# acados/acados

Measured on NVIDIA H100. Metric: OCP-QP solves/sec (fp64, batch) chain-mass N=40, higher is better.
Workload: dtype f64

## Files before the change

### acados_b200/csrc/cuipm_fast_core.h

```cpp
#ifndef CUIPM_FAST_CORE_H_
#define CUIPM_FAST_CORE_H_

#include "cuipm_device.h"

#ifndef FK_PROF_T0
#define FK_PROF_T0() do {} while (0)
#define FK_PROF_ADD(slot) do {} while (0)
#define FK_PROF_T2() do {} while (0)
#define FK_PROF_ADD2(slot) do {} while (0)
#endif

#define FK_FOR_SLACK(i, jj) \
    _Pragma("unroll 1") for (int i_ = inv[jj], i = i_ >= 0 ? i_ : 0, e_ = i_ >= 0 ? i_ + 1 : (i_ == -2 ? nb : 0); i < e_; i++) \
        if (i_ >= 0 || rev[i] == (jj))

#define FK_PRAGMA_(x) _Pragma(#x)
#define FK_PRAGMA(x) FK_PRAGMA_(x)
#ifndef FK_VLOOP_N
#define FK_VLOOP_N 1
#endif
#define FK_VLOOP FK_PRAGMA(unroll FK_VLOOP_N)
#ifndef FK_TILE_N
#define FK_TILE_LOOP _Pragma("unroll")
#else
// ... 10 lines not shown
#ifndef FK_U_TRMM
#define FK_U_TRMM 4
#endif
#ifndef FK_U_SYRK
#define FK_U_SYRK 3
#endif
#ifndef FK_U_UPD
#define FK_U_UPD 2
#endif

namespace cuipm {
namespace fastk {

FK_DEV int evn(int n) { return (n + 1) & ~1; }

struct QpState
{
    double mu, obj, gap, alpha, res_m_tau;
    double res_max[4];
};

template <int NX, int NU, int G>
struct Ker
{
    static constexpr int NM = NX + NU;
    static constexpr int QPW = 32 / G;
    static constexpr int LDK = NM | 1;
    static constexpr int LDW = ((NM + 1) / 4) * 4 + 2;
    static constexpr int RPM = (NM + G - 1) / G;
    static constexpr int NXe = (NX + 1) & ~1, NMe = (NM + 2) & ~1;
    static constexpr int SZA = (LDK * NX + 1) & ~1;
    static constexpr int SZL = LDW * NM;
    static constexpr int SZU = (NM * NU + 1) & ~1;
    static constexpr int SZD = 0;
// ... 131 lines not shown
    }
    FK_DEV void st(double *p, double v) const { if (act) *p = v; }
    template <bool ALIGNED>
    FK_DEV fk_double2 ld_pair(const double *p) const
    {
        if (ALIGNED) return fk_ld2(p);
        fk_double2 r;
        r.x = p[0]; r.y = p[1];
        return r;
    }

    template <int REC, int BAR>
    FK_DEV void bulk(int soff, size_t off, int nd, int pf = 0)
    {
        if (li == 0)
            fk_bulk(smem0 + (size_t) gq * A.gstride + soff, (REC == 0 ? qk : (REC == 1 ? sol : (REC == 2 ? wk : qp))) + off, (unsigned) nd * 8u, bars + BAR);
        (void) pf;
        if (BAR == 0) tx0 += (unsigned) (QPW * nd) * 8u;
        else tx1 += (unsigned) (QPW * nd) * 8u;
    }
    template <int REC>
    FK_DEV void vcopy(double *dst, size_t off, int nd)
    {
        const double *src = (REC == 0 ? qk : (REC == 1 ? sol : (REC == 2 ? wk : qp))) + off;
FK_VLOOP
        for (int e = 2 * li; e < nd; e += 2 * G) fk_cp16(dst + e, src + e);
    }
    FK_DEV void stage_begin() { fk_fence_async(); fk_sync(); }
    FK_DEV void stage_arm()
    {
        if (fk_lane() == 0) fk_mbar_arrive_tx(bars + 1, tx1);
        tx1 = 0;
    }
    FK_DEV void stage_arm_vec() {}
    FK_DEV void stage_arm_mat()
    {
        if (fk_lane() == 0) fk_mbar_arrive_tx(bars + 1, tx1);
        tx1 = 0;
    }
    FK_DEV void wait_vec() { FK_PROF_T0(); fk_cp_wait(); fk_sync(); FK_PROF_ADD(5); }
    FK_DEV void wait_mat() { FK_PROF_T0(); fk_mbar_wait(bars + 1, ph1); ph1 ^= 1u; FK_PROF_ADD(6); }
// ... 91 lines not shown

    FK_DEV void res_issue_mat(int k)
    {
        const StageDesc &s = sdr(k);
        const unsigned kk = (k >= 1 && k < A.N) ? (unsigned) (k - 1) : 0u;
        const int kind = k == 0 ? 0 : (k == A.N ? 2 : 1);
        if (s.nx1 > 0) bulk<0, 1>(voff(MA), (size_t) A.kq[kind] + (size_t) kk * A.kqs, evn(LDK * s.nx1));
        bulk<0, 1>(voff(ML), (size_t) A.kq[kind] + (size_t) kk * A.kqs + A.kH[kind], evn(LDK * s.n));
        stage_arm_mat();
    }

    struct ResAcc
    {
        double a_mu, a_obj, a_gap, m0, m1, m2, m3, m4;
        int f0, f1, f2, f3, f4;
    };

    template <int KIND>
    FK_DEV void res_stage(int k, int update, double alpha_u, ResAcc &R)
    {
        constexpr int nx = KD<KIND>::nx, nu = KD<KIND>::nu, n = nx + nu, nx1 = KD<KIND>::nx1;
        constexpr int RP = (n + G - 1) / G, CP = (nx1 + G - 1) / G;
        const StageDesc &sd = sdk<KIND>();
        const View v = view<KIND>(k);
        const int nb = sd.nb, ns = sd.ns, nc = sd.nc;
        const int *idxb = IDX + 4 * (A.nmaps == 3 ? KIND : k) * A.nbe, *rev = idxb + nb, *inv = rev + nb;
        const int nu1 = (nx1 > 0 && k + 1 < A.N) ? NU : 0, n1e = (nx1 + nu1 + 1) & ~1;
        const int solN = (int) (sd.sol.t - sd.sol.ux) + evn(nc), stpN = (int) (sd.step.t - sd.step.ux) + evn(nc);
        const int qvN = (int) ((sd.q_stage + sd.q_stage_bytes / 8u) - sd.q_b);
        double *SOL = V, *STP = SOL + (A.nve + NXe + 2 * A.nce), *SOLN = STP + (A.nve + NXe + 2 * A.nce), *STPN = SOLN + NMe;
        double *QV = STPN + NMe, *tmp0 = QV + (NXe + NMe + 2 * A.nce + 2 * A.ns2e), *tmp1 = tmp0 + A.nbe, *g_ = tmp1 + A.nbe, *pim = g_ + A.nve;
        double *x1 = pim + NXe;
        const int pf = (KIND == 1 && k + 1 < A.N) ? 1 : 0;
        stage_begin();
        vcopy<1>(SOL, (size_t) v.kk * A.ss + sd.sol.ux, solN);
        if (update) vcopy<2>(STP, (size_t) v.kk * A.ws + sd.step.ux, stpN);
        vcopy<0>(QV, (size_t) A.kq[KIND] + (size_t) v.kk * A.kqs + A.kV[KIND], evn(qvN));
        if (nx1 > 0)
        {
            const StageDesc &s1 = sdr(k + 1);
            const View v1 = viewr(k + 1);
            vcopy<1>(SOLN, (size_t) v1.kk * A.ss + s1.sol.ux, n1e);
            if (update) vcopy<2>(STPN, (size_t) v1.kk * A.ws + s1.step.ux, n1e);
        }
        stage_arm_vec();
        if (KIND == 0) res_issue_mat(k);
        wait_vec();
        double *ux = SOL, *pi = SOL + (sd.sol.pi - sd.sol.ux), *lam = SOL + (sd.sol.lam - sd.sol.ux), *t = SOL + (sd.sol.t - sd.sol.ux);
        const double *du = STP, *dp = STP + (sd.step.pi - sd.step.ux), *dl = STP + (sd.step.lam - sd.step.ux), *dtt = STP + (sd.step.t - sd.step.ux);
        const double *qb = QV, *qrq = QV + (sd.q_rq - sd.q_b), *qd = QV + (sd.q_d - sd.q_b), *msk = QV + (sd.q_dmask - sd.q_b);
        const double *qZ = QV + (sd.q_Z - sd.q_b), *qz = QV + (sd.q_z - sd.q_b);
        if (update)
// ... 36 lines not shown
                        tt = tt <= A.o.t_min ? A.o.t_min : tt;
                    }
                    l *= mk;
                    st(gl + i, l);
                    st(gt + i, tt);
                }
                lam[i] = l * mk;
                t[i] = tt;
            }
        }
        fk_sync();
FK_VLOOP
        for (int i = li; i < nb; i += G) tmp0[i] = lam[nb + i] - lam[i];
        wait_mat();
        fk_sync();
        {
            double hx[RPM > 0 ? RPM : 1], ap[RPM > 0 ? RPM : 1];
            rows_dot<n, n>(ML, LDK, ux, hx);
            if (nx1 > 0) rows_dot<n, nx1>(MA, LDK, pi, ap);
#pragma unroll
            for (int m = 0; m < RP; m++)
            {
                const int i = li + G * m;
                if (i < n)
                {
                    const double gv = qrq[i];
                    double r = hx[m] + 2.0 * gv;
                    R.a_obj += 0.5 * r * ux[i];
                    r -= gv;
                    R.a_gap += r * ux[i];
// ... 92 lines not shown
                R.f3 |= (a != a);
            }
            double *og = v.w + sd.res.g;
FK_VLOOP
            for (int i = li; i < n + 2 * ns; i += G)
            {
                const double r = g_[i];
                st(og + i, r);
                const double a = fabs(r);
                R.m0 = fmax(R.m0, a);
                R.f0 |= (a != a);
            }
        }
FK_VLOOP
        for (int j = li; j < nx1; j += G) pim[j] = pi[j];
    }

    FK_DEV void res_pass(int update, double alpha_u, QpState &Q)
    {
        fk_fence_async_global();

        ResAcc R;
        R.a_mu = R.a_obj = R.a_gap = R.m0 = R.m1 = R.m2 = R.m3 = R.m4 = 0.0;
        R.f0 = R.f1 = R.f2 = R.f3 = R.f4 = 0;
        if (update && alpha_u < 1.0) alpha_u = alpha_u * ((1.0 - alpha_u) * 0.99 + alpha_u * 0.9999999);
        res_stage<0>(0, update, alpha_u, R);
        for (int k = 1; k < A.N; k++) res_stage<1>(k, update, alpha_u, R);
        res_stage<2>(A.N, update, alpha_u, R);
        Q.res_max[0] = gmax_nan(R.m0, R.f0);
        Q.res_max[1] = gmax_nan(R.m1, R.f1);
        Q.res_max[2] = gmax_nan(R.m2, R.f2);
        Q.res_max[3] = gmax_nan(R.m3, R.f3);
        Q.mu = gsum(R.a_mu) * nc_mask_inv;
        Q.obj = gsum(R.a_obj);
        Q.gap = gsum(R.a_gap);
        Q.res_m_tau = gmax_nan(R.m4, R.f4);
    }

    FK_DEV void cond_slacks(int nb, int ns, const int *rev, const int *inv, const double *Z, int fact, const double *Gam, const double *gam,
                            const double *rgs, double *Zi, double *ds, double *tmp0, double *tmp1) const
    {
FK_VLOOP
        for (int j = li; j < 2 * ns; j += G)
// ... 634 lines not shown
            }
        }
    }

    FK_DEV void solve_backward(int rm_mode, double sigma_mu, bool stw)
    {
        fk_fence_async_global();

        solve_stage<2>(A.N, rm_mode, sigma_mu, stw);
        for (int k = A.N - 1; k >= 1; k--) solve_stage<1>(k, rm_mode, sigma_mu, stw);
        solve_stage<0>(0, rm_mode, sigma_mu, stw);
    }

    struct FwdAcc
    {
        double alpha, m0, m1, m2, m3;
        int f0, f1, f2, f3;
    };

    template <int KIND>
    FK_DEV void fwd_stage(int k, int after_fact, int do_lin, bool stw, FwdAcc &F)
    {
        constexpr int nx = KD<KIND>::nx, nu = KD<KIND>::nu, n = nx + nu, nx1 = KD<KIND>::nx1;
        constexpr int nsolve = nu;
        constexpr int RP = (n + G - 1) / G, CP = (nx1 + G - 1) / G;
        FK_PROF_T2();
        const StageDesc &sd = sdk<KIND>();
        const View v = view<KIND>(k);
        const int nb = sd.nb, ns = sd.ns, nc = sd.nc;
        const int *idxb = IDX + 4 * (A.nmaps == 3 ? KIND : k) * A.nbe, *rev = idxb + nb, *inv = rev + nb;
        const int nu1 = (nx1 > 0 && k + 1 < A.N) ? NU : 0, n1 = nx1 + nu1, n1e = (n1 + 1) & ~1;
        const int resN = (int) (sd.res.m - sd.res.g) + evn(nc), ltN = (int) (sd.sol.t - sd.sol.lam) + evn(nc);
        const int fvN = (int) (sd.w_Zsi - sd.w_Linv) + evn(2 * ns), qmN = (int) (sd.q_Z - sd.q_dmask) + evn(2 * ns);
        double *RES = V, *LT = RES + (A.nve + NXe + 2 * A.nce), *FV = LT + 2 * A.nce, *SUX = FV + (2 * NMe + NXe + A.ns2e), *P1 = SUX + A.nve;
        double *QM = P1 + NMe, *vv = QM + (A.nce + A.ns2e), *x1 = vv + A.nve, *tg = x1 + NXe, *pik = tg + A.nve, *pim = pik + NXe;
        double *dt = pim + NXe, *dlm = dt + A.nce, *dsv = dlm + A.nce, *tmp0 = dsv + A.ns2e;
        double *tmp = tg, *g_ = tg;
        const bool so = act && stw;
        View v1 = v;
        const StageDesc *s1p = &sd;
        if (nx1 > 0) { s1p = &sdr(k + 1); v1 = viewr(k + 1); }
        const int pf = (KIND == 1 && k + 2 < A.N) ? 1 : 0;
        stage_begin();
        vcopy<2>(RES, (size_t) v.kk * A.ws + sd.res.g, resN);
        vcopy<1>(LT, (size_t) v.kk * A.ss + sd.sol.lam, ltN);
        vcopy<2>(FV, (size_t) v.kk * A.ws + sd.w_Linv, fvN);
        vcopy<2>(SUX, (size_t) v.kk * A.ws + sd.step.ux, evn(n + 2 * ns));
        vcopy<0>(QM, (size_t) A.kq[KIND] + (size_t) v.kk * A.kqs + A.kV[KIND] + (sd.q_dmask - sd.q_b), qmN);
        if (nx1 > 0)
        {
            vcopy<2>(P1, (size_t) v1.kk * A.ws + (after_fact ? s1p->w_lrow : s1p->step.ux), n1e);
            bulk<0, 1>(voff(MA), (size_t) A.kq[KIND] + (size_t) v.kk * A.kqs, evn(LDK * nx1), pf);
        }
        if (nsolve > 0) bulk<2, 1>(voff(LU), (size_t) v.kk * A.ws + sd.w_L, evn(n * nsolve), pf);
        if (do_lin) bulk<0, 1>(voff(ML), (size_t) A.kq[KIND] + (size_t) v.kk * A.kqs + A.kH[KIND], evn(LDK * n), pf);
        else if (nx1 > 0) bulk<2, 1>(voff(ML), (size_t) v1.kk * A.ws + s1p->w_Lxx, evn((nx1 | 1) * nx1), pf);
        stage_arm();
        wait_vec();
        const double *gv = RES, *bs = RES + (sd.res.b - sd.res.g), *rds = RES + (sd.res.d - sd.res.g), *rms = RES + (sd.res.m - sd.res.g);
        const double *lam = LT, *ts = LT + (sd.sol.t - sd.sol.lam);
        const double *Lis = FV, *lrow_ = FV + (sd.w_lrow - sd.w_Linv), *Zi = FV + (sd.w_Zsi - sd.w_Linv);
        const double *mks = QM, *qZ = QM + (sd.q_Z - sd.q_dmask);
        {
            const double *src = after_fact ? lrow_ : SUX;
FK_VLOOP
            for (int i = li; i < nsolve; i += G) vv[i] = -src[i];
FK_VLOOP
            for (int j = li; j < 2 * ns; j += G) dsv[j] = SUX[n + j];
        }
        wait_mat();
        fk_sync();
        FK_PROF_ADD2(16);
        if (nsolve > 0)
        {
            double wv[NU > 0 ? NU : 1];
#pragma unroll
            for (int j = 0; j < nsolve; j++)
// ... 6 lines not shown
#pragma unroll
            for (int j = nsolve - 1; j >= 0; j--)
            {
                double part = 0.0;
#pragma unroll
                for (int i = j + 1; i < nsolve; i++) part += LU[i + n * j] * wv[i];
                wv[j] = (wv[j] - part) * Lis[j];
            }
            fk_sync();
#pragma unroll
            for (int j = 0; j < nsolve; j++)
                if (li == j % G) vv[j] = wv[j];
            fk_sync();
        }
        {
            double *o_ = v.w + sd.step.ux;
FK_VLOOP
            for (int i = li; i < n; i += G)
                if (so) o_[i] = vv[i];
        }
        FK_PROF_ADD2(17);
        double hx[RPM > 0 ? RPM : 1];
        if (do_lin)
        {
            rows_dot<n, n>(ML, LDK, vv, hx);
            if (nx1 > 0)
            {
                stage_begin();
                bulk<2, 1>(voff(ML), (size_t) v1.kk * A.ws + s1p->w_Lxx, evn((nx1 | 1) * nx1), pf);
                stage_arm_mat();
            }
        }
        FK_PROF_ADD2(18);
        if (nx1 > 0)
        {
            double av[RPM > 0 ? RPM : 1];
            cols_dot<n, nx1>(MA, LDK, vv, av);
            double *ob = v.w + sd.ires.b;
#pragma unroll
            for (int m = 0; m < CP; m++)
            {
                const int j = li + G * m;
                if (j < nx1)
                {
                    const double acc = av[m], bv = bs[j];
                    const double xj = bv + acc;
                    x1[j] = xj;
                    if (do_lin)
                    {
                        const double r = bv - xj + acc;
                        if (so) ob[j] = r;
                        const double a = fabs(r);
                        F.m1 = fmax(F.m1, a);
                        F.f1 |= (a != a);
                    }
                }
            }
        }
        FK_PROF_ADD2(19);
        {
            double *tis = dlm;
            recip_vec(ts, tis, nc);
FK_VLOOP
            for (int i = li; i < nb; i += G)
            {
                const double a = vv[idxb[i]];
                dt[i] = a;
                dt[nb + i] = -a;
            }
            if (ns > 0)
            {
                fk_sync();
                const double t_min_inv = A.o.t_min > 0 ? 1.0 / A.o.t_min : 1e30;
FK_VLOOP
                for (int j = li; j < 2 * ns; j += G)
                {
// ... 4 lines not shown
                            const double l = lam[offc + i], tt = ts[offc + i];
                            const double Gm = A.o.t_lam_min == 1 ? (tt < A.o.t_min ? t_min_inv : tis[offc + i]) * (l < A.o.lam_min ? A.o.lam_min : l) : tis[offc + i] * l;
                            d += Gm * dt[offc + i];
                        }
                    d = -Zi[j] * d;
                    dsv[j] = d;
                    dt[2 * nb + j] = d;
                }
                fk_sync();
FK_VLOOP
                for (int i = li; i < 2 * nb; i += G)
                {
                    const int up = i >= nb, ii = up ? i - nb : i;
                    if (rev[ii] >= 0) dt[i] += dsv[(up ? ns : 0) + rev[ii]];
                }
                double *o_ = v.w + sd.step.ux + n;
FK_VLOOP
                for (int j = li; j < 2 * ns; j += G)
                    if (so) o_[j] = dsv[j];
            }
            fk_sync();
            double *odl = v.w + sd.step.lam, *odt = v.w + sd.step.t, *ld_ = v.w + sd.ires.d, *lm_ = v.w + sd.ires.m;
FK_VLOOP
            for (int i = li; i < nc; i += G)
            {
                const double l = lam[i], tt = ts[i], ti = tis[i], rdi = rds[i], rmi = rms[i];
                const double dtr = dt[i];
                double dl = -ti * (rmi + (l * dtr) - (l * rdi));
                double dti = dtr - rdi;
                const double mk = mks[i];
                dl *= mk;
                dti *= mk;
                if (so) { odl[i] = dl; odt[i] = dti; }
                dlm[i] = dl * mk;
                if (l + dl < 0.0) F.alpha = fmin(F.alpha, -l / dl);
                if (tt + dti < 0.0) F.alpha = fmin(F.alpha, -tt / dti);
                if (do_lin)
                {
                    double r = (dti + rdi) - dtr;
                    r *= mk;
                    if (so) ld_[i] = r;
                    double a = fabs(r);
                    F.m2 = fmax(F.m2, a);
                    F.f2 |= (a != a);
                    double mm = rmi + l * dti + dl * tt;
                    mm *= mk;
                    if (so) lm_[i] = mm;
                    a = fabs(mm);
                    F.m3 = fmax(F.m3, a);
                    F.f3 |= (a != a);
                }
            }
        }
        FK_PROF_ADD2(20);
        if (nx1 > 0)
        {
            if (do_lin) wait_mat();
            fk_sync();
            const double *Lx = ML;
            constexpr int ldx = nx1 | 1;
            double tt_[RPM > 0 ? RPM : 1];
            cols_dot<nx1, nx1>(Lx, ldx, x1, tt_);
#pragma unroll
            for (int m = 0; m < CP; m++)
            {
                const int j = li + G * m;
                if (j < nx1) tmp[j] = after_fact ? tt_[m] + P1[nu1 + j] : tt_[m];
            }
            fk_sync();
            double *pi = v.w + sd.step.pi;
            rows_dot<nx1, nx1>(Lx, ldx, tmp, tt_);
#pragma unroll
            for (int m = 0; m < CP; m++)
            {
                const int i = li + G * m;
                if (i < nx1)
                {
                    const double pv = after_fact ? tt_[m] : tt_[m] + P1[nu1 + i];
                    if (so) pi[i] = pv;
                    pik[i] = pv;
                }
            }
        }
        fk_sync();
        FK_PROF_ADD2(21);
        if (do_lin)
        {
FK_VLOOP
            for (int i = li; i < nb; i += G) tmp0[i] = dlm[nb + i] - dlm[i];
            double ap[RPM > 0 ? RPM : 1];
            if (nx1 > 0) rows_dot<n, nx1>(MA, LDK, pik, ap);
#pragma unroll
            for (int m = 0; m < RP; m++)
            {
                const int i = li + G * m;
                if (i < n)
                {
                    double r = hx[m] + gv[i];
                    if (nx > 0 && i >= nu) r -= pim[i - nu];
                    if (nx1 > 0) r += ap[m];
                    g_[i] = r;
                }
            }
            fk_sync();
FK_VLOOP
            for (int i = li; i < nb; i += G) g_[idxb[i]] += tmp0[i];
            if (ns > 0)
            {
                const double *zv = gv + n;
FK_VLOOP
                for (int j = li; j < 2 * ns; j += G)
                {
                    double r = qZ[j] * dsv[j] + zv[j] - dlm[2 * nb + j];
                    const int jj = j < ns ? j : j - ns, offl = j < ns ? 0 : nb;
                    FK_FOR_SLACK(i, jj) r -= dlm[offl + i];
                    g_[n + j] = r;
                }
            }
            fk_sync();
            double *og = v.w + sd.ires.g;
FK_VLOOP
            for (int i = li; i < n + 2 * ns; i += G)
            {
                const double r = g_[i];
                if (so) og[i] = r;
                const double a = fabs(r);
                F.m0 = fmax(F.m0, a);
                F.f0 |= (a != a);
            }
        }
        FK_PROF_ADD2(22);
        if (nx1 > 0)
        {
FK_VLOOP
            for (int j = li; j < nx1; j += G)
            {
                vv[nu1 + j] = x1[j];
                pim[j] = pik[j];
            }
        }
    }

    FK_DEV double forward_pass(int after_fact, int do_lin, bool stw, double lin_nrm[4])
    {
        fk_fence_async_global();

        FwdAcc F;
        F.alpha = 1.0;
        F.m0 = F.m1 = F.m2 = F.m3 = 0.0;
        F.f0 = F.f1 = F.f2 = F.f3 = 0;
        fwd_stage<0>(0, after_fact, do_lin, stw, F);
        for (int k = 1; k < A.N; k++) fwd_stage<1>(k, after_fact, do_lin, stw, F);
        fwd_stage<2>(A.N, after_fact, do_lin, stw, F);
        if (do_lin)
        {
            lin_nrm[0] = gmax_nan(F.m0, F.f0);
            lin_nrm[1] = gmax_nan(F.m1, F.f1);
            lin_nrm[2] = gmax_nan(F.m2, F.f2);
            lin_nrm[3] = gmax_nan(F.m3, F.f3);
        }
        return gmin(F.alpha);
    }

    FK_DEV double mu_aff_pass(double alpha)
    {
        const int N = A.N;
        double acc = 0.0;
        auto plain = [&](int k) {
            const StageDesc &s = sdr(k);
            const View v = viewr(k);
            const double *l = v.s + s.sol.lam, *t = v.s + s.sol.t, *dl = v.w + s.step.lam, *dt = v.w + s.step.t;
// ... 209 lines not shown
            if (li == 0)
            {
                info->status = status;
                info->iter = kk;
                for (int i = 0; i < 4; i++) info->res_max[i] = Q.res_max[i];
                info->mu = Q.mu;
                info->obj = Q.obj;
                info->dual_gap = Q.gap;
                info->lq_count = 0;
                info->reserved = 0;
            }
            act = false;
        }
    }

    FK_DEV void iteration(int q, int kk, QpState &Q, cuipm_info *info, double *stat)
    {
        const int SM = CUIPM_STAT_M;
        double *stt = (stat && kk + 1 < A.o.stat_max) ? stat + SM * (size_t) (kk + 1) : nullptr;
        double nrm[4] = {0, 0, 0, 0};
        double alpha = 1.0, mu_aff = 0.0, sigma_mu = 0.0;
        bool need = true;
        for (int ph = 0; ph < 3; ph++)
        {
            const bool stw = ph < 2 ? true : need;
            { FK_PROF_T0(); if (ph == 0) fact_backward(); else solve_backward(ph, sigma_mu, stw); FK_PROF_ADD(ph == 0 ? 1 : 3); }
            const int do_lin = ph == 0 ? A.o.lq_fact == 1 : A.o.itref_corr_max > 0;
            double nr[4] = {0, 0, 0, 0};
            double al; { FK_PROF_T0(); al = forward_pass(ph == 0, do_lin, stw, nr); FK_PROF_ADD(2); }
            if (stw) { alpha = al; nrm[0] = nr[0]; nrm[1] = nr[1]; nrm[2] = nr[2]; nrm[3] = nr[3]; }
            if (ph == 0)
            {
                if (A.o.lq_fact == 1)
                {
                    const double g00 = (wk + A.s0.ires.g)[0];
                    if ((nrm[0] == 0.0 && g00 != g00) || nrm[0] > 1e-5 || nrm[1] > 1e-5 || nrm[2] > 1e-5 || nrm[3] > 1e-5)
                        if (act) { hand_back(q, info); act = false; }
                }
                if (stt && act && li == 0) { stt[13] = 0; stt[0] = alpha; stt[1] = alpha; }
                if (A.o.pred_corr != 1) break;
            }
            else if (ph == 2 || A.o.cond_pred_corr != 1)
                break;
            const double mu_aff0 = mu_aff;
            { FK_PROF_T0(); mu_aff = mu_aff_pass(alpha); FK_PROF_ADD(4); }
            if (ph == 0)
            {
                const double tmp = mu_aff / Q.mu;
                const double sigma = tmp * tmp * tmp;
                sigma_mu = sigma * Q.mu;
                sigma_mu = sigma_mu > A.o.tau_min ? sigma_mu : A.o.tau_min;
                if (stt && act && li == 0) { stt[2] = mu_aff; stt[3] = sigma; }
            }
            else
            {
                need = mu_aff > 2.0 * mu_aff0;
                if (!fk_any(act && need)) break;
            }
        }
        if (A.o.pred_corr == 1)
        {
            if (A.o.itref_corr_max > 0)
            {
                const bool small_ = (nrm[0] < A.o.res_g_max || nrm[0] < 1e-3 * Q.res_max[0]) && (nrm[1] < A.o.res_b_max || nrm[1] < 1e-3 * Q.res_max[1])
                                    && (nrm[2] < A.o.res_d_max || nrm[2] < 1e-3 * Q.res_max[2]) && (nrm[3] < A.o.res_m_max || nrm[3] < 1e-3 * Q.res_max[3]);
                if (!small_ && act) { hand_back(q, info); act = false; }
                if (stt && act && li == 0) { stt[16] = nrm[0]; stt[17] = nrm[1]; stt[18] = nrm[2]; stt[19] = nrm[3]; }
            }
            if (stt && act && li == 0) { stt[4] = alpha; stt[5] = alpha; }
        }
        if (stt && act && li == 0) stt[15] = 0;
        Q.alpha = alpha;
    }

    FK_DEV void solve(int q, bool valid)
    {
        const int SM = CUIPM_STAT_M;
        bind(q, valid);
        cuipm_info *info = A.info + q;
        double *stat = A.stat ? A.stat + (size_t) q * SM * (A.o.stat_max + 1) : nullptr;
        QpState Q;
        Q.mu = Q.obj = Q.gap = 0.0; Q.alpha = 1.0; Q.res_m_tau = 0.0;
        Q.res_max[0] = Q.res_max[1] = Q.res_max[2] = Q.res_max[3] = 0.0;
        prologue(q, info, stat);
        for (int kk = 0;; kk++)
        {
            { FK_PROF_T0(); res_pass(kk > 0, Q.alpha, Q); FK_PROF_ADD(0); }
            close_pass(kk, Q, info, stat);
            if (!fk_any(act)) break;
            iteration(q, kk, Q, info, stat);
        }
    }

    static constexpr int RRS = 12;
    static constexpr int RRK = CUIPM_RR_RINGS;
    FK_DEV static int rr_bucket(double mu)
    {
        int b = 0;
        double th = 0.1;
#pragma unroll
        for (int i = 0; i < RRK - 1; i++) { b += mu < th; th *= 0.1; }
        return b;
    }
    FK_DEV void rr_save(int q, int kk, const QpState &Q) const
    {
// ... 52 lines not shown
        fk_sync();
    }

    FK_DEV void rr_first(int first_qp)
    {
        const int SM = CUIPM_STAT_M;
        int q = first_qp + gq;
        const bool valid = q < A.nbatch;
        if (!valid) q = A.nbatch - 1;
        bind(q, valid);
        cuipm_info *info = A.info + q;
        double *stat = A.stat ? A.stat + (size_t) q * SM * (A.o.stat_max + 1) : nullptr;
        QpState Q;
        Q.mu = Q.obj = Q.gap = 0.0; Q.alpha = 1.0; Q.res_m_tau = 0.0;
        Q.res_max[0] = Q.res_max[1] = Q.res_max[2] = Q.res_max[3] = 0.0;
        prologue(q, info, stat);
        res_pass(0, 1.0, Q);
        close_pass(0, Q, info, stat);
        rr_publish(q, valid, 0, Q);
        fk_sync();
    }

    FK_DEV void rr_loop()
    {
        const int SM = CUIPM_STAT_M;
        unsigned nap = 4000;
        for (;;)
        {
            int cnt = 0;
            size_t myslot = 0;
            bool mine = false;
            for (int b = 0; b < RRK && cnt < QPW; b++)
// ... 29 lines not shown
            {
                int d = fk_lane() == 0 ? fk_ld_volatile(A.rr_ctr + 2 * RRK) : 0;
                d = fk_any(d >= A.nbatch) ? 1 : 0;
                if (d) break;
                fk_nanosleep(nap);
                if (nap < 128000) nap *= 2;
                continue;
            }
            nap = 4000;
            fk_threadfence();
            if (!have) q = 0;
            bind(q, have);
            cuipm_info *info = A.info + q;
            double *stat = A.stat ? A.stat + (size_t) q * SM * (A.o.stat_max + 1) : nullptr;
            QpState Q;
            int kk = rr_load(q, Q);
            fk_sync();
            iteration(q, kk, Q, info, stat);
            kk++;
            { FK_PROF_T0(); res_pass(1, Q.alpha, Q); FK_PROF_ADD(0); }
            close_pass(kk, Q, info, stat);
            rr_publish(q, have, kk, Q);
        }
    }

    FK_DEV void hand_back(int q, cuipm_info *info)
    {
        if (li == 0)
        {
            info->status = CUIPM_FAST_REDO;
            const int slot = fk_atomic_inc(A.redo_count);
            A.redo_list[slot] = q;
        }
    }
};

inline int vector_pool_doubles(int NX, int NM, int nce, int nbe, int ns2e, int nve)
{
    const int nxe = (NX + 1) & ~1, nme = (NM + 2) & ~1;
    const int img = nve + nxe + 2 * nce;
    const int v_res = 2 * img + 2 * nme + (nxe + nme + 2 * nce + 2 * ns2e) + 2 * nbe + nve + 2 * nxe;
    const int dd8 = 72 - (2 * nce + 2 * nbe + 2 * ns2e) > 0 ? 72 - (2 * nce + 2 * nbe + 2 * ns2e) : 0;
    const int v_fact = img + 2 * nce + ns2e + 2 * nce + 2 * nbe + 2 * ns2e + dd8 + 2 * nme + nxe + nme + nxe;
    const int v_slv = img + 2 * nce + (2 * nme + nxe + ns2e) + nce + 2 * nce + (nce + ns2e) + 2 * nce + 2 * nbe + ns2e + 2 * nxe;
    const int v_fwd = img + 2 * nce + (2 * nme + nxe + ns2e) + nve + nme + (nce + ns2e) + nve + nxe + nve + 2 * nxe + 2 * nce + ns2e + nbe;
    const int v_init = nve + nce, v_mu = 16 * nce;
    int m = v_res;
    if (v_mu > m) m = v_mu;
    if (v_fact > m) m = v_fact;
    if (v_slv > m) m = v_slv;
    if (v_fwd > m) m = v_fwd;
    if (v_init > m) m = v_init;
    return m + 8;
}

}
}
#endif
```

### acados_b200/csrc/cuipm_plan.h

```cpp
#ifndef CUIPM_PLAN_H_
#define CUIPM_PLAN_H_

#include <algorithm>
#include <cstring>
#include <string>
#include <vector>

#include "cuipm.h"
#include "cuipm_device.h"

namespace cuipm {

static inline unsigned plan_ev2u(size_t n) { return (unsigned) ((n + 1) & ~(size_t) 1); }

inline int build_plan(const cuipm_shape *sh, const cuipm_layout *l, std::vector<StageDesc> &sd, std::vector<int> &ipool, ProbDesc &P,
                      std::string &err)
{
    const int N = sh->N;
    ipool.clear();
    sd.assign(N + 1, StageDesc{});
    P = ProbDesc{};
    P.N = N;
    size_t w = 0;
    for (int k = 0; k <= N; k++)
// ... 90 lines not shown
    bool same_maps = true;
    for (int k = 1; k <= N - 1; k++)
    {
        const StageDesc &d = sd[k];
        if (d.nx != a.nx || d.nu != a.nu || d.nb != a.nb || d.ns != a.ns) return false;
        for (int i = 0; i < 2 * a.nb; i++)
            if (ipool[d.idx_off + i] != ipool[a.idx_off + i]) same_maps = false;
        const unsigned dq = qs * (unsigned) (k - 1), dsol = ss * (unsigned) (k - 1), dw = ws * (unsigned) (k - 1);
        bool ok = d.idx_off == a.idx_off + is * (k - 1);
        ok = ok && d.q_BAt == a.q_BAt + dq && d.q_RSQ == a.q_RSQ + dq && d.q_b == a.q_b + dq && d.q_rq == a.q_rq + dq && d.q_d == a.q_d + dq
             && d.q_dmask == a.q_dmask + dq && d.q_Z == a.q_Z + dq && d.q_z == a.q_z + dq && d.q_stage == a.q_stage + dq;
        ok = ok && d.sol.ux == a.sol.ux + dsol && d.sol.pi == a.sol.pi + dsol && d.sol.lam == a.sol.lam + dsol && d.sol.t == a.sol.t + dsol;
        ok = ok && d.w_L == a.w_L + dw && d.w_Linv == a.w_Linv + dw && d.w_lrow == a.w_lrow + dw && d.w_Pb == a.w_Pb + dw && d.w_Zsi == a.w_Zsi + dw && d.w_Lxx == a.w_Lxx + dw
             && d.step.ux == a.step.ux + dw && d.step.pi == a.step.pi + dw && d.step.lam == a.step.lam + dw && d.step.t == a.step.t + dw
             && d.res.g == a.res.g + dw && d.res.b == a.res.b + dw && d.res.d == a.res.d + dw && d.res.m == a.res.m + dw && d.w_rmb == a.w_rmb + dw
             && d.itref.pi == a.itref.pi + dw && d.itref.lam == a.itref.lam + dw && d.itref.t == a.itref.t + dw;
        if (!ok) return false;
    }
    F.N = N;
    F.nct = P.nct;
    F.nmaps = same_maps ? 3 : N + 1;
    F.s0 = sd[0]; F.s1 = sd[1]; F.sN = sd[N];
    F.qs = qs; F.ss = ss; F.ws = ws; F.is = is;
    F.qp_stride = P.qp_stride; F.sol_stride = P.sol_stride; F.work_stride = P.work_stride; F.w_bkp = P.w_bkp;
    auto e = [](int n) { return (n + 1) & ~1; };
    F.nce = e(P.ncmax); F.nbe = e(P.nbgmax); F.ns2e = e(2 * P.nsmax); F.nve = e(P.nvsmax);
    const int NM = a.nx + a.nu;
    F.ld = NM | 1;
    unsigned o = 0;
    const StageDesc *three[3] = {&sd[0], &sd[1], &sd[N]};
// ... 36 lines not shown
```

Measured before the change: 72060.

## Defer linear-system residual g-check from forward pass into next residual pass

Result: faster. 79720, median of 6 (+10.6%).

```diff
diff --git a/acados_b200/csrc/cuipm_fast_core.h b/acados_b200/csrc/cuipm_fast_core.h
--- a/acados_b200/csrc/cuipm_fast_core.h
+++ b/acados_b200/csrc/cuipm_fast_core.h
@@ -2,6 +2,10 @@
 #define CUIPM_FAST_CORE_H_
 
 #include "cuipm_device.h"
+
+#ifndef FK_COUNT_STAGED
+#define FK_COUNT_STAGED(bytes) do {} while (0)
+#endif
 
 #ifndef FK_PROF_T0
 #define FK_PROF_T0() do {} while (0)
@@ -48,10 +52,25 @@
 
 FK_DEV int evn(int n) { return (n + 1) & ~1; }
 
+FK_DEV double mul_rn(double a, double b)
+{
+#ifdef __CUDA_ARCH__
+    return __dmul_rn(a, b);
+#else
+    return a * b;
+#endif
+}
+
 struct QpState
 {
     double mu, obj, gap, alpha, res_m_tau;
     double res_max[4];
+};
+
+struct LinNrm
+{
+    double aff_g, fin_g, res0_g;
+    bool aff_bdm_large, fin_bdm_small;
 };
 
 template <int NX, int NU, int G>
@@ -213,7 +232,10 @@
     FK_DEV void bulk(int soff, size_t off, int nd, int pf = 0)
     {
         if (li == 0)
+        {
             fk_bulk(smem0 + (size_t) gq * A.gstride + soff, (REC == 0 ? qk : (REC == 1 ? sol : (REC == 2 ? wk : qp))) + off, (unsigned) nd * 8u, bars + BAR);
+            FK_COUNT_STAGED((unsigned) nd * 8u);
+        }
         (void) pf;
         if (BAR == 0) tx0 += (unsigned) (QPW * nd) * 8u;
         else tx1 += (unsigned) (QPW * nd) * 8u;
@@ -223,7 +245,11 @@
     {
         const double *src = (REC == 0 ? qk : (REC == 1 ? sol : (REC == 2 ? wk : qp))) + off;
 FK_VLOOP
-        for (int e = 2 * li; e < nd; e += 2 * G) fk_cp16(dst + e, src + e);
+        for (int e = 2 * li; e < nd; e += 2 * G)
+        {
+            fk_cp16(dst + e, src + e);
+            FK_COUNT_STAGED(16u);
+        }
     }
     FK_DEV void stage_begin() { fk_fence_async(); fk_sync(); }
     FK_DEV void stage_arm()
@@ -345,10 +371,51 @@
     {
         double a_mu, a_obj, a_gap, m0, m1, m2, m3, m4;
         int f0, f1, f2, f3, f4;
+        double ma, mf, pa[RPM > 0 ? RPM : 1], pf[RPM > 0 ? RPM : 1];
+        int fa, ff;
     };
 
     template <int KIND>
-    FK_DEV void res_stage(int k, int update, double alpha_u, ResAcc &R)
+    FK_DEV void lin_rows(const double *du, const double *dp, const double *dl, bool mask_dl, const double *msk, const double *rg,
+                         const double *qZ, const int *idxb, const int *rev, const int *inv, int nb, int ns, const double (&pm)[RPM > 0 ? RPM : 1],
+                         double &mx, int &fl) const
+    {
+        constexpr int nx = KD<KIND>::nx, nu = KD<KIND>::nu, n = nx + nu, nx1 = KD<KIND>::nx1;
+        constexpr int RP = (n + G - 1) / G;
+        double hx[RPM > 0 ? RPM : 1], ap[RPM > 0 ? RPM : 1];
+        rows_dot<n, n>(ML, LDK, du, hx);
+        if (nx1 > 0) rows_dot<n, nx1>(MA, LDK, dp, ap);
+#pragma unroll
+        for (int m = 0; m < RP; m++)
+        {
+            const int i = li + G * m;
+            if (i < n)
+            {
+                double r = hx[m] + rg[i];
+                if (nx > 0 && i >= nu) r -= pm[m];
+                if (nx1 > 0) r += ap[m];
+                for (int b = 0; b < nb; b++)
+                    if (idxb[b] == i)
+                        r += (mask_dl ? mul_rn(dl[nb + b], msk[nb + b]) : dl[nb + b]) - (mask_dl ? mul_rn(dl[b], msk[b]) : dl[b]);
+                const double a = fabs(r);
+                mx = fmax(mx, a);
+                fl |= (a != a);
+            }
+        }
+FK_VLOOP
+        for (int j = li; j < 2 * ns; j += G)
+        {
+            double r = qZ[j] * du[n + j] + rg[n + j] - (mask_dl ? mul_rn(dl[2 * nb + j], msk[2 * nb + j]) : dl[2 * nb + j]);
+            const int jj = j < ns ? j : j - ns, offl = j < ns ? 0 : nb;
+            FK_FOR_SLACK(i, jj) r -= mask_dl ? mul_rn(dl[offl + i], msk[offl + i]) : dl[offl + i];
+            const double a = fabs(r);
+            mx = fmax(mx, a);
+            fl |= (a != a);
+        }
+    }
+
+    template <int KIND>
+    FK_DEV void res_stage(int k, int update, bool lin_a, bool lin_f, double alpha_u, ResAcc &R)
     {
         constexpr int nx = KD<KIND>::nx, nu = KD<KIND>::nu, n = nx + nu, nx1 = KD<KIND>::nx1;
         constexpr int RP = (n + G - 1) / G, CP = (nx1 + G - 1) / G;
@@ -361,12 +428,14 @@
         const int qvN = (int) ((sd.q_stage + sd.q_stage_bytes / 8u) - sd.q_b);
         double *SOL = V, *STP = SOL + (A.nve + NXe + 2 * A.nce), *SOLN = STP + (A.nve + NXe + 2 * A.nce), *STPN = SOLN + NMe;
         double *QV = STPN + NMe, *tmp0 = QV + (NXe + NMe + 2 * A.nce + 2 * A.ns2e), *tmp1 = tmp0 + A.nbe, *g_ = tmp1 + A.nbe, *pim = g_ + A.nve;
-        double *x1 = pim + NXe;
+        double *x1 = pim + NXe, *AF = x1 + NXe;
         const int pf = (KIND == 1 && k + 1 < A.N) ? 1 : 0;
         stage_begin();
         vcopy<1>(SOL, (size_t) v.kk * A.ss + sd.sol.ux, solN);
         if (update) vcopy<2>(STP, (size_t) v.kk * A.ws + sd.step.ux, stpN);
         vcopy<0>(QV, (size_t) A.kq[KIND] + (size_t) v.kk * A.kqs + A.kV[KIND], evn(qvN));
+        if (lin_a || lin_f) vcopy<2>(g_, (size_t) v.kk * A.ws + sd.res.g, evn(n + 2 * ns));
+        if (lin_a) vcopy<2>(AF, (size_t) v.kk * A.ws + sd.ires.g, (int) (sd.ires.d - sd.ires.g) + evn(nc));
         if (nx1 > 0)
         {
             const StageDesc &s1 = sdr(k + 1);
@@ -433,6 +502,8 @@
         for (int i = li; i < nb; i += G) tmp0[i] = lam[nb + i] - lam[i];
         wait_mat();
         fk_sync();
+        if (lin_a) lin_rows<KIND>(AF, AF + (sd.ires.b - sd.ires.g), AF + (sd.ires.d - sd.ires.g), false, msk, g_, qZ, idxb, rev, inv, nb, ns, R.pa, R.ma, R.fa);
+        if (lin_f) lin_rows<KIND>(du, dp, dl, true, msk, g_, qZ, idxb, rev, inv, nb, ns, R.pf, R.mf, R.ff);
         {
             double hx[RPM > 0 ? RPM : 1], ap[RPM > 0 ? RPM : 1];
             rows_dot<n, n>(ML, LDK, ux, hx);
@@ -555,19 +626,39 @@
         }
 FK_VLOOP
         for (int j = li; j < nx1; j += G) pim[j] = pi[j];
-    }
-
-    FK_DEV void res_pass(int update, double alpha_u, QpState &Q)
+        if (nx1 > 0 && (lin_a || lin_f))
+        {
+            const int nun = k + 1 < A.N ? NU : 0;
+            const double *dpa = AF + (sd.ires.b - sd.ires.g);
+#pragma unroll
+            for (int m = 0; m < RPM; m++)
+            {
+                const int j = li + G * m - nun;
+                const bool in = j >= 0 && j < nx1;
+                R.pa[m] = in && lin_a ? dpa[j] : 0.0;
+                R.pf[m] = in && lin_f ? dp[j] : 0.0;
+            }
+        }
+    }
+
+    FK_DEV void res_pass(int update, double alpha_u, QpState &Q, LinNrm &L)
     {
         fk_fence_async_global();
 
+        const bool lin_a = update && A.o.lq_fact == 1, lin_f = update && A.o.pred_corr == 1 && A.o.itref_corr_max > 0;
         ResAcc R;
         R.a_mu = R.a_obj = R.a_gap = R.m0 = R.m1 = R.m2 = R.m3 = R.m4 = 0.0;
         R.f0 = R.f1 = R.f2 = R.f3 = R.f4 = 0;
+        R.ma = R.mf = 0.0;
+        R.fa = R.ff = 0;
+#pragma unroll
+        for (int m = 0; m < (RPM > 0 ? RPM : 1); m++) R.pa[m] = R.pf[m] = 0.0;
         if (update && alpha_u < 1.0) alpha_u = alpha_u * ((1.0 - alpha_u) * 0.99 + alpha_u * 0.9999999);
-        res_stage<0>(0, update, alpha_u, R);
-        for (int k = 1; k < A.N; k++) res_stage<1>(k, update, alpha_u, R);
-        res_stage<2>(A.N, update, alpha_u, R);
+        res_stage<0>(0, update, lin_a, lin_f, alpha_u, R);
+        for (int k = 1; k < A.N; k++) res_stage<1>(k, update, lin_a, lin_f, alpha_u, R);
+        res_stage<2>(A.N, update, lin_a, lin_f, alpha_u, R);
+        if (lin_a) L.aff_g = gmax_nan(R.ma, R.fa);
+        if (lin_f) L.fin_g = gmax_nan(R.mf, R.ff);
         Q.res_max[0] = gmax_nan(R.m0, R.f0);
         Q.res_max[1] = gmax_nan(R.m1, R.f1);
         Q.res_max[2] = gmax_nan(R.m2, R.f2);
@@ -1232,8 +1323,8 @@
 
     struct FwdAcc
     {
-        double alpha, m0, m1, m2, m3;
-        int f0, f1, f2, f3;
+        double alpha, m1, m2, m3;
+        int f1, f2, f3;
     };
 
     template <int KIND>
@@ -1241,44 +1332,42 @@
     {
         constexpr int nx = KD<KIND>::nx, nu = KD<KIND>::nu, n = nx + nu, nx1 = KD<KIND>::nx1;
         constexpr int nsolve = nu;
-        constexpr int RP = (n + G - 1) / G, CP = (nx1 + G - 1) / G;
+        constexpr int CP = (nx1 + G - 1) / G;
         FK_PROF_T2();
         const StageDesc &sd = sdk<KIND>();
         const View v = view<KIND>(k);
         const int nb = sd.nb, ns = sd.ns, nc = sd.nc;
         const int *idxb = IDX + 4 * (A.nmaps == 3 ? KIND : k) * A.nbe, *rev = idxb + nb, *inv = rev + nb;
         const int nu1 = (nx1 > 0 && k + 1 < A.N) ? NU : 0, n1 = nx1 + nu1, n1e = (n1 + 1) & ~1;
-        const int resN = (int) (sd.res.m - sd.res.g) + evn(nc), ltN = (int) (sd.sol.t - sd.sol.lam) + evn(nc);
-        const int fvN = (int) (sd.w_Zsi - sd.w_Linv) + evn(2 * ns), qmN = (int) (sd.q_Z - sd.q_dmask) + evn(2 * ns);
+        const int resN = (int) (sd.res.m - sd.res.b) + evn(nc), ltN = (int) (sd.sol.t - sd.sol.lam) + evn(nc);
+        const int fvN = (int) (sd.w_Zsi - sd.w_Linv) + evn(2 * ns);
         double *RES = V, *LT = RES + (A.nve + NXe + 2 * A.nce), *FV = LT + 2 * A.nce, *SUX = FV + (2 * NMe + NXe + A.ns2e), *P1 = SUX + A.nve;
-        double *QM = P1 + NMe, *vv = QM + (A.nce + A.ns2e), *x1 = vv + A.nve, *tg = x1 + NXe, *pik = tg + A.nve, *pim = pik + NXe;
-        double *dt = pim + NXe, *dlm = dt + A.nce, *dsv = dlm + A.nce, *tmp0 = dsv + A.ns2e;
-        double *tmp = tg, *g_ = tg;
-        const bool so = act && stw;
+        double *QM = P1 + NMe, *vv = QM + (A.nce + A.ns2e), *x1 = vv + A.nve, *tmp = x1 + NXe;
+        double *dt = tmp + A.nve, *tis = dt + A.nce, *dsv = tis + A.nce;
+        const bool so = act && stw, sa = so && after_fact && do_lin;
         View v1 = v;
         const StageDesc *s1p = &sd;
         if (nx1 > 0) { s1p = &sdr(k + 1); v1 = viewr(k + 1); }
         const int pf = (KIND == 1 && k + 2 < A.N) ? 1 : 0;
         stage_begin();
-        vcopy<2>(RES, (size_t) v.kk * A.ws + sd.res.g, resN);
+        vcopy<2>(RES, (size_t) v.kk * A.ws + sd.res.b, resN);
         vcopy<1>(LT, (size_t) v.kk * A.ss + sd.sol.lam, ltN);
         vcopy<2>(FV, (size_t) v.kk * A.ws + sd.w_Linv, fvN);
         vcopy<2>(SUX, (size_t) v.kk * A.ws + sd.step.ux, evn(n + 2 * ns));
-        vcopy<0>(QM, (size_t) A.kq[KIND] + (size_t) v.kk * A.kqs + A.kV[KIND] + (sd.q_dmask - sd.q_b), qmN);
+        vcopy<0>(QM, (size_t) A.kq[KIND] + (size_t) v.kk * A.kqs + A.kV[KIND] + (sd.q_dmask - sd.q_b), evn(nc));
         if (nx1 > 0)
         {
             vcopy<2>(P1, (size_t) v1.kk * A.ws + (after_fact ? s1p->w_lrow : s1p->step.ux), n1e);
             bulk<0, 1>(voff(MA), (size_t) A.kq[KIND] + (size_t) v.kk * A.kqs, evn(LDK * nx1), pf);
         }
         if (nsolve > 0) bulk<2, 1>(voff(LU), (size_t) v.kk * A.ws + sd.w_L, evn(n * nsolve), pf);
-        if (do_lin) bulk<0, 1>(voff(ML), (size_t) A.kq[KIND] + (size_t) v.kk * A.kqs + A.kH[KIND], evn(LDK * n), pf);
-        else if (nx1 > 0) bulk<2, 1>(voff(ML), (size_t) v1.kk * A.ws + s1p->w_Lxx, evn((nx1 | 1) * nx1), pf);
+        if (nx1 > 0) bulk<2, 1>(voff(ML), (size_t) v1.kk * A.ws + s1p->w_Lxx, evn((nx1 | 1) * nx1), pf);
         stage_arm();
         wait_vec();
-        const double *gv = RES, *bs = RES + (sd.res.b - sd.res.g), *rds = RES + (sd.res.d - sd.res.g), *rms = RES + (sd.res.m - sd.res.g);
+        const double *bs = RES, *rds = RES + (sd.res.d - sd.res.b), *rms = RES + (sd.res.m - sd.res.b);
         const double *lam = LT, *ts = LT + (sd.sol.t - sd.sol.lam);
         const double *Lis = FV, *lrow_ = FV + (sd.w_lrow - sd.w_Linv), *Zi = FV + (sd.w_Zsi - sd.w_Linv);
-        const double *mks = QM, *qZ = QM + (sd.q_Z - sd.q_dmask);
+        const double *mks = QM;
         {
             const double *src = after_fact ? lrow_ : SUX;
 FK_VLOOP
@@ -1315,29 +1404,19 @@
             fk_sync();
         }
         {
-            double *o_ = v.w + sd.step.ux;
+            double *o_ = v.w + sd.step.ux, *oa = v.w + sd.ires.g;
 FK_VLOOP
             for (int i = li; i < n; i += G)
+            {
                 if (so) o_[i] = vv[i];
+                if (sa) oa[i] = vv[i];
+            }
         }
         FK_PROF_ADD2(17);
-        double hx[RPM > 0 ? RPM : 1];
-        if (do_lin)
-        {
-            rows_dot<n, n>(ML, LDK, vv, hx);
-            if (nx1 > 0)
-            {
-                stage_begin();
-                bulk<2, 1>(voff(ML), (size_t) v1.kk * A.ws + s1p->w_Lxx, evn((nx1 | 1) * nx1), pf);
-                stage_arm_mat();
-            }
-        }
-        FK_PROF_ADD2(18);
         if (nx1 > 0)
         {
             double av[RPM > 0 ? RPM : 1];
             cols_dot<n, nx1>(MA, LDK, vv, av);
-            double *ob = v.w + sd.ires.b;
 #pragma unroll
             for (int m = 0; m < CP; m++)
             {
@@ -1350,7 +1429,6 @@
                     if (do_lin)
                     {
                         const double r = bv - xj + acc;
-                        if (so) ob[j] = r;
                         const double a = fabs(r);
                         F.m1 = fmax(F.m1, a);
                         F.f1 |= (a != a);
@@ -1360,7 +1438,6 @@
         }
         FK_PROF_ADD2(19);
         {
-            double *tis = dlm;
             recip_vec(ts, tis, nc);
 FK_VLOOP
             for (int i = li; i < nb; i += G)
@@ -1395,13 +1472,16 @@
                     const int up = i >= nb, ii = up ? i - nb : i;
                     if (rev[ii] >= 0) dt[i] += dsv[(up ? ns : 0) + rev[ii]];
                 }
-                double *o_ = v.w + sd.step.ux + n;
+                double *o_ = v.w + sd.step.ux + n, *oa = v.w + sd.ires.g + n;
 FK_VLOOP
                 for (int j = li; j < 2 * ns; j += G)
+                {
                     if (so) o_[j] = dsv[j];
+                    if (sa) oa[j] = dsv[j];
+                }
             }
             fk_sync();
-            double *odl = v.w + sd.step.lam, *odt = v.w + sd.step.t, *ld_ = v.w + sd.ires.d, *lm_ = v.w + sd.ires.m;
+            double *odl = v.w + sd.step.lam, *odt = v.w + sd.step.t, *oa = v.w + sd.ires.d;
 FK_VLOOP
             for (int i = li; i < nc; i += G)
             {
@@ -1413,20 +1493,18 @@
                 dl *= mk;
                 dti *= mk;
                 if (so) { odl[i] = dl; odt[i] = dti; }
-                dlm[i] = dl * mk;
+                if (sa) oa[i] = dl * mk;
                 if (l + dl < 0.0) F.alpha = fmin(F.alpha, -l / dl);
                 if (tt + dti < 0.0) F.alpha = fmin(F.alpha, -tt / dti);
                 if (do_lin)
                 {
                     double r = (dti + rdi) - dtr;
                     r *= mk;
-                    if (so) ld_[i] = r;
                     double a = fabs(r);
                     F.m2 = fmax(F.m2, a);
                     F.f2 |= (a != a);
                     double mm = rmi + l * dti + dl * tt;
                     mm *= mk;
-                    if (so) lm_[i] = mm;
                     a = fabs(mm);
                     F.m3 = fmax(F.m3, a);
                     F.f3 |= (a != a);
@@ -1436,7 +1514,6 @@
         FK_PROF_ADD2(20);
         if (nx1 > 0)
         {
-            if (do_lin) wait_mat();
             fk_sync();
             const double *Lx = ML;
             constexpr int ldx = nx1 | 1;
@@ -1449,7 +1526,7 @@
                 if (j < nx1) tmp[j] = after_fact ? tt_[m] + P1[nu1 + j] : tt_[m];
             }
             fk_sync();
-            double *pi = v.w + sd.step.pi;
+            double *pi = v.w + sd.step.pi, *oa = v.w + sd.ires.b;
             rows_dot<nx1, nx1>(Lx, ldx, tmp, tt_);
 #pragma unroll
             for (int m = 0; m < CP; m++)
@@ -1459,66 +1536,16 @@
                 {
                     const double pv = after_fact ? tt_[m] : tt_[m] + P1[nu1 + i];
                     if (so) pi[i] = pv;
-                    pik[i] = pv;
+                    if (sa) oa[i] = pv;
                 }
             }
         }
         fk_sync();
         FK_PROF_ADD2(21);
-        if (do_lin)
-        {
-FK_VLOOP
-            for (int i = li; i < nb; i += G) tmp0[i] = dlm[nb + i] - dlm[i];
-            double ap[RPM > 0 ? RPM : 1];
-            if (nx1 > 0) rows_dot<n, nx1>(MA, LDK, pik, ap);
-#pragma unroll
-            for (int m = 0; m < RP; m++)
-            {
-                const int i = li + G * m;
-                if (i < n)
-                {
-                    double r = hx[m] + gv[i];
-                    if (nx > 0 && i >= nu) r -= pim[i - nu];
-                    if (nx1 > 0) r += ap[m];
-                    g_[i] = r;
-                }
-            }
-            fk_sync();
-FK_VLOOP
-            for (int i = li; i < nb; i += G) g_[idxb[i]] += tmp0[i];
-            if (ns > 0)
-            {
-                const double *zv = gv + n;
-FK_VLOOP
-                for (int j = li; j < 2 * ns; j += G)
-                {
-                    double r = qZ[j] * dsv[j] + zv[j] - dlm[2 * nb + j];
-                    const int jj = j < ns ? j : j - ns, offl = j < ns ? 0 : nb;
-                    FK_FOR_SLACK(i, jj) r -= dlm[offl + i];
-                    g_[n + j] = r;
-                }
-            }
-            fk_sync();
-            double *og = v.w + sd.ires.g;
-FK_VLOOP
-            for (int i = li; i < n + 2 * ns; i += G)
-            {
-                const double r = g_[i];
-                if (so) og[i] = r;
-                const double a = fabs(r);
-                F.m0 = fmax(F.m0, a);
-                F.f0 |= (a != a);
-            }
-        }
-        FK_PROF_ADD2(22);
         if (nx1 > 0)
         {
 FK_VLOOP
-            for (int j = li; j < nx1; j += G)
-            {
-                vv[nu1 + j] = x1[j];
-                pim[j] = pik[j];
-            }
+            for (int j = li; j < nx1; j += G) vv[nu1 + j] = x1[j];
         }
     }
 
@@ -1528,14 +1555,13 @@
 
         FwdAcc F;
         F.alpha = 1.0;
-        F.m0 = F.m1 = F.m2 = F.m3 = 0.0;
-        F.f0 = F.f1 = F.f2 = F.f3 = 0;
+        F.m1 = F.m2 = F.m3 = 0.0;
+        F.f1 = F.f2 = F.f3 = 0;
         fwd_stage<0>(0, after_fact, do_lin, stw, F);
         for (int k = 1; k < A.N; k++) fwd_stage<1>(k, after_fact, do_lin, stw, F);
         fwd_stage<2>(A.N, after_fact, do_lin, stw, F);
         if (do_lin)
         {
-            lin_nrm[0] = gmax_nan(F.m0, F.f0);
             lin_nrm[1] = gmax_nan(F.m1, F.f1);
             lin_nrm[2] = gmax_nan(F.m2, F.f2);
             lin_nrm[3] = gmax_nan(F.m3, F.f3);
@@ -1775,7 +1801,7 @@
         }
     }
 
-    FK_DEV void iteration(int q, int kk, QpState &Q, cuipm_info *info, double *stat)
+    FK_DEV void iteration(int q, int kk, QpState &Q, LinNrm &L, cuipm_info *info, double *stat)
     {
         const int SM = CUIPM_STAT_M;
         double *stt = (stat && kk + 1 < A.o.stat_max) ? stat + SM * (size_t) (kk + 1) : nullptr;
@@ -1789,15 +1815,10 @@
             const int do_lin = ph == 0 ? A.o.lq_fact == 1 : A.o.itref_corr_max > 0;
             double nr[4] = {0, 0, 0, 0};
             double al; { FK_PROF_T0(); al = forward_pass(ph == 0, do_lin, stw, nr); FK_PROF_ADD(2); }
-            if (stw) { alpha = al; nrm[0] = nr[0]; nrm[1] = nr[1]; nrm[2] = nr[2]; nrm[3] = nr[3]; }
+            if (stw) { alpha = al; nrm[1] = nr[1]; nrm[2] = nr[2]; nrm[3] = nr[3]; }
             if (ph == 0)
             {
-                if (A.o.lq_fact == 1)
-                {
-                    const double g00 = (wk + A.s0.ires.g)[0];
-                    if ((nrm[0] == 0.0 && g00 != g00) || nrm[0] > 1e-5 || nrm[1] > 1e-5 || nrm[2] > 1e-5 || nrm[3] > 1e-5)
-                        if (act) { hand_back(q, info); act = false; }
-                }
+                L.aff_bdm_large = nr[1] > 1e-5 || nr[2] > 1e-5 || nr[3] > 1e-5;
                 if (stt && act && li == 0) { stt[13] = 0; stt[0] = alpha; stt[1] = alpha; }
                 if (A.o.pred_corr != 1) break;
             }
@@ -1823,15 +1844,30 @@
         {
             if (A.o.itref_corr_max > 0)
             {
-                const bool small_ = (nrm[0] < A.o.res_g_max || nrm[0] < 1e-3 * Q.res_max[0]) && (nrm[1] < A.o.res_b_max || nrm[1] < 1e-3 * Q.res_max[1])
-                                    && (nrm[2] < A.o.res_d_max || nrm[2] < 1e-3 * Q.res_max[2]) && (nrm[3] < A.o.res_m_max || nrm[3] < 1e-3 * Q.res_max[3]);
-                if (!small_ && act) { hand_back(q, info); act = false; }
-                if (stt && act && li == 0) { stt[16] = nrm[0]; stt[17] = nrm[1]; stt[18] = nrm[2]; stt[19] = nrm[3]; }
+                L.res0_g = Q.res_max[0];
+                L.fin_bdm_small = (nrm[1] < A.o.res_b_max || nrm[1] < 1e-3 * Q.res_max[1]) && (nrm[2] < A.o.res_d_max || nrm[2] < 1e-3 * Q.res_max[2])
+                                  && (nrm[3] < A.o.res_m_max || nrm[3] < 1e-3 * Q.res_max[3]);
+                if (stt && act && li == 0) { stt[17] = nrm[1]; stt[18] = nrm[2]; stt[19] = nrm[3]; }
             }
             if (stt && act && li == 0) { stt[4] = alpha; stt[5] = alpha; }
         }
         if (stt && act && li == 0) stt[15] = 0;
         Q.alpha = alpha;
+    }
+
+    FK_DEV void lin_check(int q, int kk, const LinNrm &L, cuipm_info *info, double *stat)
+    {
+        if (A.o.lq_fact == 1)
+        {
+            if (L.aff_g > 1e-5 || L.aff_bdm_large)
+                if (act) { hand_back(q, info); act = false; }
+        }
+        if (A.o.pred_corr == 1 && A.o.itref_corr_max > 0)
+        {
+            const bool small_ = (L.fin_g < A.o.res_g_max || L.fin_g < 1e-3 * L.res0_g) && L.fin_bdm_small;
+            if (!small_ && act) { hand_back(q, info); act = false; }
+            if (stat && kk < A.o.stat_max && act && li == 0) stat[CUIPM_STAT_M * (size_t) kk + 16] = L.fin_g;
+        }
     }
 
     FK_DEV void solve(int q, bool valid)
@@ -1843,13 +1879,15 @@
         QpState Q;
         Q.mu = Q.obj = Q.gap = 0.0; Q.alpha = 1.0; Q.res_m_tau = 0.0;
         Q.res_max[0] = Q.res_max[1] = Q.res_max[2] = Q.res_max[3] = 0.0;
+        LinNrm L;
         prologue(q, info, stat);
         for (int kk = 0;; kk++)
         {
-            { FK_PROF_T0(); res_pass(kk > 0, Q.alpha, Q); FK_PROF_ADD(0); }
+            { FK_PROF_T0(); res_pass(kk > 0, Q.alpha, Q, L); FK_PROF_ADD(0); }
+            if (kk > 0) lin_check(q, kk, L, info, stat);
             close_pass(kk, Q, info, stat);
             if (!fk_any(act)) break;
-            iteration(q, kk, Q, info, stat);
+            iteration(q, kk, Q, L, info, stat);
         }
     }
 
@@ -1932,8 +1970,9 @@
         QpState Q;
         Q.mu = Q.obj = Q.gap = 0.0; Q.alpha = 1.0; Q.res_m_tau = 0.0;
         Q.res_max[0] = Q.res_max[1] = Q.res_max[2] = Q.res_max[3] = 0.0;
+        LinNrm L;
         prologue(q, info, stat);
-        res_pass(0, 1.0, Q);
+        res_pass(0, 1.0, Q, L);
         close_pass(0, Q, info, stat);
         rr_publish(q, valid, 0, Q);
         fk_sync();
@@ -1993,11 +2032,13 @@
             cuipm_info *info = A.info + q;
             double *stat = A.stat ? A.stat + (size_t) q * SM * (A.o.stat_max + 1) : nullptr;
             QpState Q;
+            LinNrm L;
             int kk = rr_load(q, Q);
             fk_sync();
-            iteration(q, kk, Q, info, stat);
+            iteration(q, kk, Q, L, info, stat);
             kk++;
-            { FK_PROF_T0(); res_pass(1, Q.alpha, Q); FK_PROF_ADD(0); }
+            { FK_PROF_T0(); res_pass(1, Q.alpha, Q, L); FK_PROF_ADD(0); }
+            lin_check(q, kk, L, info, stat);
             close_pass(kk, Q, info, stat);
             rr_publish(q, have, kk, Q);
         }
@@ -2018,11 +2059,11 @@
 {
     const int nxe = (NX + 1) & ~1, nme = (NM + 2) & ~1;
     const int img = nve + nxe + 2 * nce;
-    const int v_res = 2 * img + 2 * nme + (nxe + nme + 2 * nce + 2 * ns2e) + 2 * nbe + nve + 2 * nxe;
+    const int v_res = 2 * img + 2 * nme + (nxe + nme + 2 * nce + 2 * ns2e) + 2 * nbe + nve + 2 * nxe + (nve + nxe + nce);
     const int dd8 = 72 - (2 * nce + 2 * nbe + 2 * ns2e) > 0 ? 72 - (2 * nce + 2 * nbe + 2 * ns2e) : 0;
     const int v_fact = img + 2 * nce + ns2e + 2 * nce + 2 * nbe + 2 * ns2e + dd8 + 2 * nme + nxe + nme + nxe;
     const int v_slv = img + 2 * nce + (2 * nme + nxe + ns2e) + nce + 2 * nce + (nce + ns2e) + 2 * nce + 2 * nbe + ns2e + 2 * nxe;
-    const int v_fwd = img + 2 * nce + (2 * nme + nxe + ns2e) + nve + nme + (nce + ns2e) + nve + nxe + nve + 2 * nxe + 2 * nce + ns2e + nbe;
+    const int v_fwd = img + 2 * nce + (2 * nme + nxe + ns2e) + nve + nme + (nce + ns2e) + nve + nxe + nve + 2 * nce + ns2e;
     const int v_init = nve + nce, v_mu = 16 * nce;
     int m = v_res;
     if (v_mu > m) m = v_mu;
diff --git a/acados_b200/csrc/cuipm_plan.h b/acados_b200/csrc/cuipm_plan.h
--- a/acados_b200/csrc/cuipm_plan.h
+++ b/acados_b200/csrc/cuipm_plan.h
@@ -128,6 +128,7 @@
         ok = ok && d.w_L == a.w_L + dw && d.w_Linv == a.w_Linv + dw && d.w_lrow == a.w_lrow + dw && d.w_Pb == a.w_Pb + dw && d.w_Zsi == a.w_Zsi + dw && d.w_Lxx == a.w_Lxx + dw
              && d.step.ux == a.step.ux + dw && d.step.pi == a.step.pi + dw && d.step.lam == a.step.lam + dw && d.step.t == a.step.t + dw
              && d.res.g == a.res.g + dw && d.res.b == a.res.b + dw && d.res.d == a.res.d + dw && d.res.m == a.res.m + dw && d.w_rmb == a.w_rmb + dw
+             && d.ires.g == a.ires.g + dw && d.ires.b == a.ires.b + dw && d.ires.d == a.ires.d + dw
              && d.itref.pi == a.itref.pi + dw && d.itref.lam == a.itref.lam + dw && d.itref.t == a.itref.t + dw;
         if (!ok) return false;
     }
```
